# taleinat/fuzzysearch

Hardware: AMD Instinct MI355X
Metric: GB/s of sequence scanned at |p|=20 max_l_dist=2 (levenshtein_ngram path; two searches in flight: see value_sync for one synchronous call at a time) (higher is better)
Workload: dtype u8

## Files before the change

fuzzysearch_amd/_native.py:

```python
import ctypes
import os
import threading

_HERE = os.path.dirname(os.path.abspath(__file__))
LIB_PATH = os.environ.get("FUZZYSEARCH_HIP_LIB") or os.path.join(_HERE, "libfzhip.so")

FZ_OK, FZ_EINVAL, FZ_ENOMEM, FZ_EDEVICE, FZ_EUNSUPPORTED, FZ_EHALO, FZ_ETIMEOUT = 0, -1, -2, -3, -4, -5, -6
UINT64_MAX = (1 << 64) - 1

EXPORTED_SYMBOLS = (
    "fz_abi_version", "fz_last_error", "fz_device_count", "fz_create", "fz_destroy",
    "fz_seq_upload", "fz_seq_upload_shard", "fz_seq_new", "fz_seq_add_shard", "fz_seq_len", "fz_seq_release",
    "fz_search_exact", "fz_lev_ngrams", "fz_lev_ngrams_begin", "fz_lev_ngrams_end", "fz_subs_ngrams", "fz_generic_ngrams",
    "fz_subs_ngrams_begin", "fz_generic_ngrams_begin", "fz_search_end",
    "fz_lev_lp", "fz_subs_lp", "fz_generic_lp", "fz_subs_ngrams_any", "fz_subs_lp_any", "fz_generic_ngrams_any", "fz_generic_ngrams_consolidated",
    "fz_lev_ngrams_consolidated", "fz_subs_ngrams_best",
    "fz_stream_open", "fz_stream_buffer", "fz_stream_submit", "fz_stream_read_fd", "fz_stream_finish", "fz_stream_close",
    "fz_consolidate", "fz_group_best", "fz_merge_ranks", "fz_wire_pack", "fz_wire_merge", "fz_debug_launch_plan", "fz_debug_order_records", "fz_debug_order_records_bounded", "fz_debug_order_segments", "fz_stats", "fz_mem_info", "fz_set_timing", "fz_set_streams", "fz_device_ms", "fz_free",
    "fz_comm_unique_id", "fz_comm_init_rank", "fz_comm_init_all", "fz_comm_info", "fz_comm_set_collective",
    "fz_comm_allgather", "fz_comm_max_f64", "fz_comm_barrier", "fz_comm_destroy", "fz_comm_gather_ms", "fz_comm_backend", "fz_debug_reload_switches", "fz_debug_gather_merge", "fz_debug_scan_regions",
)


class FzMatch(ctypes.Structure):
    _fields_ = [("start", ctypes.c_int64), ("end", ctypes.c_int64),
                ("dist", ctypes.c_int32), ("block", ctypes.c_int32)]


class FzStats(ctypes.Structure):
    _fields_ = [("bytes_scanned", ctypes.c_uint64), ("ngram_hits", ctypes.c_uint64),
                ("raw_matches", ctypes.c_uint64), ("filter_ms", ctypes.c_double),
                ("verify_ms", ctypes.c_double), ("device_ms", ctypes.c_double),
                ("filter_launches", ctypes.c_uint32), ("n_devices", ctypes.c_uint32),
                ("verify_form", ctypes.c_uint32), ("reserved_", ctypes.c_uint32)]


FORM_NONE, FORM_FUSED_BAND, FORM_FUSED_CELLS, FORM_FUSED_BITS1, FORM_FUSED_BITS2, FORM_KERNEL, FORM_FUSED_BITS32 = range(7)


class HipEngineError(RuntimeError):
    """libfzhip.so missing / no usable gfx950 device / HIP runtime failure."""


class CollectiveTimeout(HipEngineError):
    """A collective of the context's communicator did not complete within FZ_COMM_TIMEOUT_MS (a rank never arrived)."""


_lib = None
_lib_lock = threading.Lock()


def load_library():
    global _lib
# ... 25 lines not shown
        L.fz_seq_upload_shard.argtypes = [vp, u8p, u64, u64, u64, u64, u64, ctypes.POINTER(vp)]
        L.fz_seq_new.restype = ci
        L.fz_seq_new.argtypes = [vp, u64, ctypes.POINTER(vp)]
        L.fz_seq_add_shard.restype = ci
        L.fz_seq_add_shard.argtypes = [vp, ci, u8p, u64, u64, u64, u64]
        L.fz_device_ms.restype = ci
        L.fz_device_ms.argtypes = [vp, ctypes.POINTER(ctypes.c_double), ci]
        L.fz_comm_unique_id.restype = ci
        L.fz_comm_unique_id.argtypes = [vp, u64]
        L.fz_comm_init_rank.restype = ci
        L.fz_comm_init_rank.argtypes = [vp, vp, ci, ci]
        L.fz_comm_init_all.restype = ci
        L.fz_comm_init_all.argtypes = [vp]
        L.fz_comm_info.restype = ci
        L.fz_comm_info.argtypes = [vp, ctypes.POINTER(ci), ctypes.POINTER(ci), ctypes.POINTER(ci)]
        L.fz_comm_set_collective.restype = ci
        L.fz_comm_set_collective.argtypes = [vp, ci]
        L.fz_comm_allgather.restype = ci
        L.fz_comm_allgather.argtypes = [vp, vp, u64, vp]
        L.fz_comm_max_f64.restype = ci
        L.fz_comm_max_f64.argtypes = [vp, ctypes.POINTER(ctypes.c_double)]
        L.fz_comm_barrier.restype = ci
        L.fz_comm_barrier.argtypes = [vp]
        L.fz_comm_destroy.restype = None
        L.fz_comm_destroy.argtypes = [vp]
        L.fz_debug_reload_switches.restype = None
        L.fz_debug_reload_switches.argtypes = []
        L.fz_comm_backend.restype = ci
        L.fz_comm_backend.argtypes = []
        L.fz_comm_gather_ms.restype = ci
        L.fz_comm_gather_ms.argtypes = [vp, ctypes.POINTER(ctypes.c_double)]
        L.fz_debug_scan_regions.restype = ci
        L.fz_debug_scan_regions.argtypes = [u64, u64, u32, ci, ctypes.c_double, ci, ctypes.POINTER(u32), ctypes.c_void_p]
        L.fz_debug_gather_merge.restype = ci
        L.fz_debug_gather_merge.argtypes = [ctypes.c_void_p, u32, u64, ctypes.c_void_p, u32, mpp, u64p, u64p]
        L.fz_seq_len.restype = u64
        L.fz_seq_len.argtypes = [vp]
        L.fz_seq_release.restype = None
        L.fz_seq_release.argtypes = [vp]
        L.fz_search_exact.restype = ci
        L.fz_search_exact.argtypes = [vp, vp, u8p, u32, u64, u64, ctypes.POINTER(u64p), u64p]
        L.fz_lev_ngrams.restype = ci
        L.fz_lev_ngrams.argtypes = [vp, vp, u8p, u32, u32, mpp, u64p]
        L.fz_lev_ngrams_begin.restype = ci
        L.fz_lev_ngrams_begin.argtypes = [vp, vp, u8p, u32, u32]
        L.fz_lev_ngrams_end.restype = ci
        L.fz_lev_ngrams_end.argtypes = [vp, mpp, u64p]
        L.fz_search_end.restype = ci
        L.fz_search_end.argtypes = [vp, mpp, u64p]
        L.fz_subs_ngrams_begin.restype = ci
        L.fz_subs_ngrams_begin.argtypes = [vp, vp, u8p, u32, u32]
        L.fz_generic_ngrams_begin.restype = ci
        L.fz_generic_ngrams_begin.argtypes = [vp, vp, u8p, u32, u32, u32, u32, u32, ci]
        L.fz_subs_ngrams.restype = ci
        L.fz_subs_ngrams.argtypes = [vp, vp, u8p, u32, u32, mpp, u64p]
        L.fz_generic_ngrams.restype = ci
        L.fz_generic_ngrams.argtypes = [vp, vp, u8p, u32, u32, u32, u32, u32, mpp, u64p]
        L.fz_lev_lp.restype = ci
        L.fz_lev_lp.argtypes = [vp, vp, u8p, u32, u32, mpp, u64p]
        L.fz_subs_lp.restype = ci
        L.fz_subs_lp.argtypes = [vp, vp, u8p, u32, u32, mpp, u64p]
        L.fz_generic_lp.restype = ci
        L.fz_generic_lp.argtypes = [vp, vp, u8p, u32, u32, u32, u32, u32, mpp, u64p]
        L.fz_lev_ngrams_consolidated.restype = ci
        L.fz_lev_ngrams_consolidated.argtypes = [vp, vp, u8p, u32, u32, mpp, u64p]
        L.fz_subs_ngrams_best.restype = ci
# ... 587 lines not shown
```

fuzzysearch_amd/csrc/fzhip.hip:

```cpp
#include <hip/hip_runtime.h>
#include <hip/hip_ext.h>
#include <rccl/rccl.h>
#include <dlfcn.h>

#include <algorithm>
#include <atomic>
#include <chrono>
#include <condition_variable>
#include <cstdarg>
#include <cstdio>
#include <cstdlib>
#include <cstring>
#include <functional>
#include <new>
#include <string>
#include <thread>
#include <unistd.h>
#include <map>
#include <mutex>
#include <vector>
#include <cassert>

#include "../../include/fzhip.h"
#include "fz_kernels.h"
// ... 110 lines not shown
    bool dedup_zeroed = false;
    uint64_t gen_dedup_arg = 0;
    bool dedup_used = false;
    bool gen_multi_used = false;
    uint64_t gen_rows_cap = 0;
    uint8_t *h_big = nullptr;
    uint64_t big_cap = 0;
    uint8_t *spare_alloc = nullptr;
    uint64_t spare_bytes = 0;
    uint64_t first_copy = 512;
    bool header_zeroed = false;
    bool verify_launched = false;
    int scan_end_event = 1;
    int verify_end_event = 2;
    uint8_t *stream_h[2] = {nullptr, nullptr};
    uint8_t *stream_d = nullptr;
    uint64_t stream_cap = 0, stream_d_bytes = 0;
    int n_cus = 256;
    uint64_t hit_cap_used = 0, rec_cap_used = 0;
    bool fused_used = false;
    uint32_t form_used = 0;
    bool timed = true;
    double last_filter_ms = 0;
    uint64_t fold_guess = 8192, fold_copied = 0;
    bool fold_direct = true;
    bool fold_was_direct = false;
    int lp_end_event = 2;
    uint8_t *d_pat = nullptr;
    uint64_t pat_cap = 0;
    int slot_id = 0;
    uint32_t launches_used = 0;
    hipStream_t stream_alt = nullptr;
    uint8_t *d_hdr_alt = nullptr;
    ncclComm_t comm = nullptr;
    int comm_rank = -1;
    hipStream_t comm_stream = nullptr;
    uint8_t *d_send[2] = {nullptr, nullptr};
    uint64_t send_cap = 0;
    uint8_t *d_recv = nullptr, *h_recv = nullptr;
    uint64_t recv_bytes = 0;
    hipEvent_t ev_snap[2] = {nullptr, nullptr}, ev_done = nullptr;
    bool snap_taken[2] = {false, false};
    struct Slot {
        hipEvent_t ev[4] = {nullptr, nullptr, nullptr, nullptr};
        uint8_t *h_stage = nullptr, *h_stage_dev = nullptr;
        bool last_direct = false, verify_launched = false, fused_used = false, timed = true;
        int scan_end_event = 1, verify_end_event = 2;
        uint64_t hit_cap_used = 0, rec_cap_used = 0;
        int slot_id = 1;
    } other;
    void swap_slot() {
        std::swap(slot_id, other.slot_id);
        for (int i = 0; i < 4; ++i) std::swap(ev[i], other.ev[i]);
        std::swap(h_stage, other.h_stage);
        std::swap(h_stage_dev, other.h_stage_dev);
        std::swap(last_direct, other.last_direct);
        std::swap(verify_launched, other.verify_launched);
        std::swap(timed, other.timed);
        std::swap(fused_used, other.fused_used);
        std::swap(scan_end_event, other.scan_end_event);
        std::swap(verify_end_event, other.verify_end_event);
        std::swap(hit_cap_used, other.hit_cap_used);
        std::swap(rec_cap_used, other.rec_cap_used);
    }
};

struct Shard {
    int dev = 0;
    uint8_t *d_alloc = nullptr;
    uint8_t *d_buf = nullptr;
    uint64_t alloc_bytes = 0;
    FzGeom geom{};
};

}

namespace {

struct DevWorkers {
    struct W {
        std::thread th;
        std::mutex mu;
        std::condition_variable cv;
        std::function<int()> job;
        std::atomic<uint64_t> posted{0}, done{0};
        int rc = 0;
        std::string err;
        bool stop = false;
    };
    std::vector<W *> ws;
    static constexpr long kSpinUs = 1500;

// ... 447 lines not shown
        nw[j] = j + 1 < steps ? per : T - per * (steps - 1);
        weight += f[j] * (double)nw[j];
    }
    const double share = (double)ntiles / weight;
    uint64_t at = 0, wg = 0;
    auto add = [&](uint64_t nwg, uint64_t tiles) {
        fa.reg_wg0[fa.nreg] = (uint32_t)wg; fa.reg_nwg[fa.nreg] = (uint32_t)nwg;
        fa.reg_tile0[fa.nreg] = at; fa.reg_end[fa.nreg] = at + tiles;
        ++fa.nreg; wg += nwg; at += tiles;
    };
    add(Gw - T, std::min<uint64_t>(ntiles, (uint64_t)(share * (double)(Gw - T) + 0.5)));
    for (int j = 0; j < steps; ++j) {
        const uint64_t left = ntiles - at;
        add(nw[j], j + 1 < steps ? std::min<uint64_t>(left, (uint64_t)(share * f[j] * (double)nw[j] + 0.5)) : left);
    }
    for (uint32_t r = 0; r < fa.nreg; ++r)
        if ((fa.reg_end[r] - fa.reg_tile0[r] + fa.reg_nwg[r] - 1) / fa.reg_nwg[r] >= FZ_TITER_MAX) { fa.nreg = 0; break; }
}

void plan_scan_regions(FzScanArgs &fa, uint64_t ntiles, uint64_t grid, uint32_t n_cus) {
    const int steps = sw().taper_steps;
    const double fmin = sw().taper_min;
    const int t_per_cu = sw().taper_wg_per_cu;
    plan_scan_regions(fa, ntiles, grid, n_cus, steps, fmin, t_per_cu);
}

struct ScanPlan {
    uint64_t ntiles = 0;
    uint32_t grid = 1;
    int wfg = 0;
    uint32_t form = FZ_FORM_NONE;
    uint32_t lds = 0;
    VerifyPlan vp;
};

ScanPlan plan_scan(const Search &q, const FzGeom &geom, uint32_t n_cus, bool with_verify, FzScanArgs &fa) {
    ScanPlan sp;
    const uint32_t L = q.plan.L;
    const uint32_t G = (uint32_t)q.plan.s.size();
    const bool in_memory = geom.seg_stride == 0;
    const uint64_t ntiles_all = (geom.buf_len + FZ_TILE_BYTES - 1) / FZ_TILE_BYTES;
    const uint64_t tile_lo = std::min<uint64_t>(ntiles_all, q.part_lo / FZ_TILE_BYTES);
    const uint64_t tile_hi = q.part_hi == ~0ull ? ntiles_all : std::min<uint64_t>(ntiles_all, (q.part_hi + FZ_TILE_BYTES - 1) / FZ_TILE_BYTES);
    const bool partial = tile_lo != 0 || tile_hi != ntiles_all;
    const uint64_t ntiles = sp.ntiles = tile_hi > tile_lo ? tile_hi - tile_lo : 0;
    constexpr uint64_t kTilesPerWg = 12;
    const uint64_t resident = (uint64_t)n_cus * 6;
    uint64_t max_grid = std::max<uint64_t>(resident, ntiles / kTilesPerWg);
    if (ntiles < resident * 120) {
        const uint64_t rounds = std::max<uint64_t>(1, (2 * ntiles + resident * 19 / 2) / (resident * 19));
        max_grid = resident * rounds;
    }
    const uint64_t min_grid = (ntiles + FZ_TITER_MAX - 1) / FZ_TITER_MAX;
    sp.grid = (uint32_t)std::max<uint64_t>(std::max<uint64_t>(1, min_grid), std::min<uint64_t>(ntiles, max_grid));
    plan_scan_regions(fa, ntiles, sp.grid, n_cus);
    if (partial) {
        fa.nreg = 1;
        fa.reg_wg0[0] = 0; fa.reg_nwg[0] = sp.grid; fa.reg_tile0[0] = tile_lo; fa.reg_end[0] = tile_hi;
    }

    const bool force_big = sw().force_big_verify;
    sp.vp = plan_verify(q);
    const VerifyPlan &vp = sp.vp;
    fa.band_w = q.mode == FZ_MODE_LEV ? 2 * q.k + 2 : 0;
    fa.win_dwords = (q.m + 2 * q.k + 6) / 4 + 1;
    const uint32_t mpad = (q.m + 15u) & ~15u;
    constexpr uint32_t target = 18u * 1024u;
    fa.vlanes = 64;
    uint32_t fused_lds;
    if (in_memory) {
        fa.win_pieces = (q.m + 2 * q.k + 3 + 15) / 16;
        fa.qcap = 128;
        while (fa.qcap > 64 && mpad + FZ_TABLE_BYTES + FZ_WAVES_PER_BLOCK * fz_wave_lds_pref_bytes(fa.qcap, fa.win_pieces) > target + 4096)
            fa.qcap >>= 1;
        fused_lds = mpad + FZ_TABLE_BYTES + FZ_WAVES_PER_BLOCK * fz_wave_lds_pref_bytes(fa.qcap, fa.win_pieces);
        if (fa.win_pieces * 16u + 16u > FZ_PAD_BACK) fused_lds = ~0u;
    } else {
        while (fa.vlanes > 16 && mpad + FZ_TABLE_BYTES + FZ_WAVES_PER_BLOCK * fz_wave_lds_bytes(fa.win_dwords, fa.band_w, fa.vlanes, true) > target)
            fa.vlanes >>= 1;
        fused_lds = mpad + FZ_TABLE_BYTES + FZ_WAVES_PER_BLOCK * fz_wave_lds_bytes(fa.win_dwords, fa.band_w, fa.vlanes, true);
    }
    fa.fused = (with_verify && !force_big && q.m <= FZ_MAX_M && q.k <= FZ_MAX_K && fused_lds <= kFusedLdsBudget &&
                (q.mode != FZ_MODE_LEV || q.k <= 4)) ? 1u : 0u;
    int bits_nw = 0;
    double per_tile = 0;
    {
        bool seen[256] = {false};
        uint32_t sigma = 0;
        for (uint32_t i = 0; i < q.m; ++i)
            if (!seen[q.p[i]]) { seen[q.p[i]] = true; ++sigma; }
        per_tile = 4096.0 * std::min<uint32_t>(G, FZ_MAX_BLOCKS_PER_LAUNCH);
        for (uint32_t i = 0; i < L && per_tile > 0.01; ++i) per_tile /= (double)std::max(2u, sigma);
    }
// ... 4 lines not shown
        bits_nw = q.m <= FZ_BITS_MAX_M(4) ? 4 : q.m <= FZ_BITS_MAX_M(1) ? 1 : 2;
        constexpr uint32_t budget = 26u * 1024u;
        const uint32_t fixed = mpad + FZ_TABLE_BYTES + FZ_PEQ_BYTES(bits_nw);
        uint32_t qc = sw().bits_qcap > 0 ? (uint32_t)sw().bits_qcap
                                         : (uint32_t)std::min(512.0, 64.0 + 32.0 * std::ceil(2.0 * per_tile / 32.0));
        while (qc > 64u && fixed + FZ_WAVES_PER_BLOCK * fz_wave_lds_pref_bytes(qc, fa.win_pieces) > budget) qc -= 32u;
        fa.qcap = qc;
        fused_lds = fixed + FZ_WAVES_PER_BLOCK * fz_wave_lds_pref_bytes(fa.qcap, fa.win_pieces);
        if (fused_lds > kFusedLdsBudget) bits_nw = 0;
        else fa.fused = 1u;
    }
    bool adapt_plain = false;
    if (!bits_nw && fa.fused && in_memory && with_verify && !sw().no_bits && per_tile > 16.0 && q.mode == FZ_MODE_SUBS) {
        const uint32_t fixed = mpad + FZ_TABLE_BYTES;
        uint32_t qc = sw().bits_qcap > 0 ? (uint32_t)sw().bits_qcap : (uint32_t)std::min(512.0, 64.0 + 32.0 * std::ceil(2.0 * per_tile / 32.0));
        while (qc > 64u && fixed + FZ_WAVES_PER_BLOCK * fz_wave_lds_pref_bytes(qc, fa.win_pieces) > target + 4096) qc -= 32u;
        if (fixed + FZ_WAVES_PER_BLOCK * fz_wave_lds_pref_bytes(qc, fa.win_pieces) <= kFusedLdsBudget) {
            adapt_plain = true;
            fa.qcap = qc;
            fused_lds = fixed + FZ_WAVES_PER_BLOCK * fz_wave_lds_pref_bytes(qc, fa.win_pieces);
        }
    }
    const bool no_wf_fuse = sw().no_wf_fuse;
    const uint32_t wf_fused_lds = mpad + FZ_TABLE_BYTES + FZ_WAVES_PER_BLOCK * fz_wave_lds_bytes(fz_wf_fused_dwords(fa.win_dwords, (uint32_t)vp.gw), 0, 1, true);
    const int wf32_env = sw().wf32;
    const bool wf_candidate = !bits_nw && !fa.fused && in_memory && with_verify && !force_big && !no_wf_fuse && vp.want_wf && !vp.big && vp.gw <= 32 &&
                              q.m <= FZ_MAX_M && wf_fused_lds <= target + 4096;
    const bool wf_fused = wf_candidate && (vp.gw == 16 || (wf32_env >= 0 ? wf32_env != 0 : per_tile > 0.1));
    if (wf_fused) { fa.fused = 1u; fused_lds = wf_fused_lds; fa.vlanes = 64; }
    sp.wfg = bits_nw ? bits_nw : adapt_plain ? 3 : wf_fused ? vp.gw : 0;
    sp.form = !with_verify ? FZ_FORM_NONE : bits_nw == 4 ? FZ_FORM_FUSED_BITS32 : bits_nw == 1 ? FZ_FORM_FUSED_BITS1 : bits_nw == 2 ? FZ_FORM_FUSED_BITS2
              : wf_fused ? FZ_FORM_FUSED_CELLS : fa.fused ? FZ_FORM_FUSED_BAND : FZ_FORM_KERNEL;
    sp.lds = fa.fused ? fused_lds : FZ_TABLE_BYTES + FZ_WAVES_PER_BLOCK * fz_wave_lds_bytes(0, 0, 64, true);
    return sp;
}

int enqueue_shard(fz_ctx *ctx, const Shard &sh, const Search &q, bool with_verify, bool copy_back = true) {
    DevState &d = lane_dev(ctx, sh.dev);
    HIP_TRY(hipSetDevice(d.device));
    unsigned long long *counters = reinterpret_cast<unsigned long long *>(d.d_out);
    FzRec *recs = reinterpret_cast<FzRec *>(d.d_out + kHeaderBytes);
    const bool no_direct = env_no_direct();
    const bool snapshot = copy_back && with_verify && q.collective;
    const bool direct = copy_back && d.direct && !no_direct && !snapshot && sh.geom.buf_len > 0 && !q.plan.s.empty();
    if (direct && with_verify) recs = reinterpret_cast<FzRec *>(d.h_stage_dev + kHeaderBytes);
    d.last_direct = direct;
    d.timed = ctx->timing;

    FzScanArgs fa;
    fill_common_args(fa, sh, q);
    const ScanPlan sp = plan_scan(q, sh.geom, (uint32_t)d.n_cus, with_verify, fa);
    const VerifyPlan &vp = sp.vp;
    const uint32_t L = q.plan.L;
    const uint32_t G = (uint32_t)q.plan.s.size();
    const uint64_t ntiles = sp.ntiles;
    const dim3 grid(sp.grid);
    if (q.mode == FZ_MODE_GENERIC && !with_verify) fa.gen_dedup = d.gen_dedup_arg;
    {
        int rc = stage_pattern(d, fa, q.p, q.m, with_verify && vp.big);
        if (rc) return rc;
    }
    const HashGeom hgeom(L);
    const int nwin = hgeom.nwin, dh = hgeom.dh;
    fa.d2 = nwin == 2 ? std::min<uint32_t>(L, 8) - 4 : 0;
    fa.mask1 = hgeom.mask1;
    fa.mask2 = 0xffffffffu;
    fa.hit_cap = d.hit_cap;
    fa.rec_cap = direct ? kHostRecs : d.rec_cap;
    const bool alt = ctx->streams == 2 && d.slot_id == 1 && fa.fused && direct && copy_back && !fa.pat_g && sh.geom.seg_stride == 0;
    const hipStream_t st = alt ? d.stream_alt : d.stream;
    if (alt) counters = reinterpret_cast<unsigned long long *>(d.d_hdr_alt);
    else {
        if (!d.header_zeroed) HIP_TRY(hipMemsetAsync(d.d_out, 0, kHeaderBytes, d.stream));
        d.header_zeroed = false;
    }

    const bool ext_events = copy_back && direct && !(with_verify && !fa.fused) && ntiles > 0 && G > 0;
    const bool attach = ntiles > 0 && G > 0;
    if (ctx->timing && !attach) HIP_TRY(hipEventRecord(d.ev[0], st));
    uint32_t launches = 0;
    for (uint32_t g0 = 0; g0 < G && ntiles > 0;) {
        uint32_t hash_k = 0, lut_shift = 0;
        const uint32_t nblk = choose_launch_blocks(q.p, q.plan.s.data(), g0, G, L, hash_k, lut_shift);
        fa.hash_k = hash_k;
        fa.lut_shift = lut_shift;
        fa.nblk = nblk;
        fa.g0 = g0;
        for (uint32_t b = 0; b < nblk; ++b) {
            const uint8_t *ng = q.p + q.plan.s[g0 + b];
            fa.A[b] = load_le32(ng, L) & fa.mask1;
            fa.B[b] = nwin == 2 ? load_le32(ng + fa.d2, 4) : 0;
            fa.H[b] = nwin == 2 ? fz_hash_windows(fa.A[b], load_le32(ng + dh, 3), fa.hash_k) : fz_hash_short(fa.A[b], fa.hash_k);
            fa.s[b] = q.plan.s[g0 + b];
            fz_block_range(q.mode, q.m, q.k, L, fa.s[b], fa.lo_rel[b], fa.hi_sub[b]);
        }
        const bool verify_follows = with_verify && !fa.fused;
        fa.host_hdr = (direct && !verify_follows && g0 + nblk >= G) ? reinterpret_cast<uint64_t>(d.h_stage_dev) : 0;
        fa.flags = q.any ? FZ_FLAG_ANY : 0u;
        for (uint32_t b = 1; b < nblk; ++b)
            for (uint32_t c = 0; c < b; ++c)
                if (fa.H[b] == fa.H[c]) fa.flags |= FZ_FLAG_DUP_HASHES;
        ScanKernel kern = scan_kernel(nwin, dh, fa.fused != 0, sh.geom.seg_stride != 0, fa.lut_shift == 2, sp.wfg);
// ... 310 lines not shown
        }
        NCCL_TRY(rccl_api()->GroupStart());
        for (DevState &d : ctx->devs)
            NCCL_TRY(rccl_api()->AllGather(d.d_send[d.slot_id], d.d_recv, bytes, ncclChar, d.comm, d.comm_stream));
        NCCL_TRY(rccl_api()->GroupEnd());
        DevState &d0 = ctx->devs[0];
        HIP_TRY(hipSetDevice(d0.device));
        HIP_TRY(hipMemcpyAsync(d0.h_recv, d0.d_recv, (uint64_t)world * bytes, hipMemcpyDeviceToHost, d0.comm_stream));
        HIP_TRY(hipEventRecord(d0.ev_done, d0.comm_stream));
        {
            int rcw = comm_wait(d0.comm_stream, "the all-gather of the ranks' records");
            if (rcw) { if (rcw == FZ_ETIMEOUT) ctx->comm_broken = true; return rcw; }
        }
        for (size_t i = 1; i < ctx->devs.size(); ++i) {
            HIP_TRY(hipSetDevice(ctx->devs[i].device));
            int rcw = comm_wait(ctx->devs[i].comm_stream, "the all-gather of the ranks' records");
            if (rcw) { if (rcw == FZ_ETIMEOUT) ctx->comm_broken = true; return rcw; }
        }
        uint64_t top = 0, total = 0;
        parse_gathered(d0.h_recv, world, bytes, ctx->gcap, seq->rank_lo.data(), recs, ctx->seg_ends, ctx->seg_order, &top, &total);
        if (top > ctx->gcap) {
            ctx->gcap = (top + top / 4 + 1023) / 1024 * 1024;
            continue;
        }
        ctx->stats.raw_matches = total;
        const uint64_t want = std::max<uint64_t>(1024, (top + top / 4 + 1023) / 1024 * 1024);
        if (want * 2 <= ctx->gcap) ctx->gcap = want;
        ctx->last_gather_ms = std::chrono::duration<double, std::milli>(std::chrono::steady_clock::now() - t_start).count();
        return FZ_OK;
    }
    return fail(FZ_EDEVICE, "all-gather capacity kept overflowing");
}

int search_enqueue(fz_ctx *ctx, fz_seq *seq, const Search &q, bool with_verify) {
    ctx->view = nullptr;
    ctx->view_n = 0;
    ctx->rows_ready = false;
    ctx->stats.filter_launches = 0;
    ctx->stats.bytes_scanned = ctx->stats.ngram_hits = ctx->stats.raw_matches = 0;
    ctx->stats.filter_ms = ctx->stats.verify_ms = ctx->stats.device_ms = 0;
    ctx->tref.clear();
    int rc = for_each_shard(ctx, seq, [ctx, seq, &q, with_verify](size_t si) { return enqueue_shard(ctx, seq->shards[si], q, with_verify); });
    if (rc) return rc;
    for (const Shard &sh : seq->shards) {
        const DevState &d = lane_dev(ctx, sh.dev);
        ctx->stats.filter_launches += d.launches_used;
        ctx->stats.verify_form = d.form_used;
    }
    return FZ_OK;
}

int emit_matches(const FzRec *recs, size_t cnt, uint32_t L, fz_match **out, uint64_t *n, uint64_t idx_bound, uint32_t blk_bound,
                 bool may_have_empty, std::vector<fz_match> *into);

int search_collect(fz_ctx *ctx, fz_seq *seq, const Search &q, bool with_verify, std::vector<FzRec> &recs,
                   std::vector<uint64_t> &hits) {
    const size_t ns = seq->shards.size();
    if (ctx->souts.size() < ns) ctx->souts.resize(ns);
    const bool order_rows = with_verify && !q.collective && ns > 1 && !q.any && seq->shards[0].geom.seg_stride == 0;
    for (int attempt = 0; attempt < 4; ++attempt) {
        recs.clear();
        hits.clear();
        ctx->rows_ready = false;
        ctx->stats.bytes_scanned = ctx->stats.ngram_hits = ctx->stats.raw_matches = 0;
        ctx->stats.filter_ms = ctx->stats.verify_ms = ctx->stats.device_ms = 0;
        ctx->tref.clear();
        Trace tr;
        ctx->seg_ends.clear();
        ctx->seg_order.clear();
        const uint32_t L = q.plan.L, nblk = (uint32_t)q.plan.s.size();
        const uint64_t nglob = seq->n;
        const bool collective = q.collective;
        int rc = for_each_shard(ctx, seq, [ctx, seq, with_verify, ns, collective, order_rows, L, nblk, nglob](size_t si) {
            ShardOut &so = ctx->souts[si];
            int r = collect_shard(ctx, seq->shards[si], with_verify, ns == 1, so, collective);
// ... 637 lines not shown
    }
    return FZ_OK;
}

int fz_create(const int *device_ids, int n_devices, fz_ctx **out) {
    if (!out) return fail(FZ_EINVAL, "null argument");
    *out = nullptr;
    int count = 0;
    hipError_t e = hipGetDeviceCount(&count);
    if (e != hipSuccess || count <= 0)
        return fail(FZ_EDEVICE, "no HIP device available (%s)", e == hipSuccess ? "count = 0" : hipGetErrorString(e));
    (void)hipSetDeviceFlags(hipDeviceScheduleSpin);
    (void)hipGetLastError();
    std::vector<int> ids;
    if (!device_ids || n_devices <= 0) ids.push_back(0);
    else ids.assign(device_ids, device_ids + n_devices);
    fz_ctx *ctx = new (std::nothrow) fz_ctx();
    if (!ctx) return fail(FZ_ENOMEM, "out of memory");
    for (int id : ids) {
        if (id < 0 || id >= count) { fz_destroy(ctx); return fail(FZ_EINVAL, "device id %d out of range (have %d)", id, count); }
        hipDeviceProp_t prop;
        if (hipGetDeviceProperties(&prop, id) != hipSuccess) { fz_destroy(ctx); return fail(FZ_EDEVICE, "hipGetDeviceProperties failed"); }
        if (strncmp(prop.gcnArchName, "gfx950", 6) != 0) {
            fz_destroy(ctx);
            return fail(FZ_EDEVICE, "device %d is %s; libfzhip is built for gfx950 (MI355X) only", id, prop.gcnArchName);
        }
        ctx->devs.emplace_back();
        DevState &d = ctx->devs.back();
        d.device = id;
        d.n_cus = prop.multiProcessorCount > 0 ? prop.multiProcessorCount : 256;
        int rc = devstate_init(d);
        if (rc) { fz_destroy(ctx); return rc; }
    }
    if (ctx->devs.size() > 1 && !sw().no_dev_threads) {
        ctx->workers = new (std::nothrow) DevWorkers(ctx->devs.size());
        if (!ctx->workers) { fz_destroy(ctx); return fail(FZ_ENOMEM, "out of memory"); }
    }
    *out = ctx;
    return FZ_OK;
}

void fz_destroy(fz_ctx *ctx) {
    if (!ctx) return;
    delete ctx->workers;
    ctx->workers = nullptr;
    while (!ctx->live.empty()) {
        for (DevState &d : ctx->devs) { (void)hipSetDevice(d.device); if (d.stream) (void)hipStreamSynchronize(d.stream); }
        fz_seq_release(ctx->live.back());
    }
    comm_teardown(ctx);
    for (DevState &d : ctx->devs) devstate_destroy(d);
    for (DevState &d : ctx->devs2) devstate_destroy(d);
    delete ctx;
}

static int upload_one(fz_ctx *ctx, int dev_index, const uint8_t *host_buf, const FzGeom &geom, Shard &sh) {
    DevState &d = ctx->devs[dev_index];
    HIP_TRY(hipSetDevice(d.device));
    const uint64_t tiles = (geom.buf_len + FZ_TILE_BYTES - 1) / FZ_TILE_BYTES;
    const uint64_t body = std::max<uint64_t>(1, tiles) * FZ_TILE_BYTES;
    sh.dev = dev_index;
    sh.alloc_bytes = FZ_PAD_FRONT + body + FZ_PAD_BACK;
    sh.geom = geom;
    if (d.spare_alloc && d.spare_bytes >= sh.alloc_bytes && d.spare_bytes <= 4 * sh.alloc_bytes + (1u << 20)) {
        sh.d_alloc = d.spare_alloc;
        sh.alloc_bytes = d.spare_bytes;
// ... 306 lines not shown
    if (ctx && ctx->npend >= 2) return fail(FZ_EINVAL, "two searches are already in flight on this context");
    const bool generic = kind == FZ_MODE_GENERIC;
    if (ctx && ctx->npend == 1 && (ctx->pend[0].kind == FZ_MODE_GENERIC) != generic)
        return fail(FZ_EINVAL, "generic searches and Levenshtein / substitutions-only searches cannot be in flight together");
    if (!ctx || !p || m == 0) return fail(FZ_EINVAL, "bad ctx / empty subsequence");
    fz_ctx::Pending &pd = ctx->pend[ctx->npend];
    pd.pattern.assign(p, p + m);
    pd.seq = seq;
    pd.m = m;
    pd.k = k;
    pd.kind = kind;
    pd.max_subs = max_subs; pd.max_ins = max_ins; pd.max_dels = max_dels;
    pd.consolidated = consolidated;
    pd.lane = 0;
    Search q;
    int rc = pending_plan(ctx, pd, q);
    if (rc) return rc;
    memset(&ctx->stats, 0, sizeof ctx->stats); ctx->tref.clear();
    ctx->stats.n_devices = (uint32_t)ctx->devs.size();
    const bool second = ctx->npend == 1;
    pd.launched = true;
    if (generic) {
        pd.lane = second ? 1 - ctx->pend[0].lane : 0;
        if (pd.lane == 1) { rc = ensure_lane2(ctx); if (rc) return rc; }
        std::vector<FzGenRec> none;
        ctx->lane = pd.lane;
        rc = run_generic(ctx, seq, q, none, 1);
        ctx->lane = 0;
        if (rc) return rc;
    } else {
        if (second && !ctx->snapshot) for (const DevState &d : ctx->devs) if (!d.direct || env_no_direct()) pd.launched = false;
        if (pd.launched) {
            if (second) for (DevState &d : ctx->devs) d.swap_slot();
            rc = search_enqueue(ctx, seq, q, true);
            if (second) for (DevState &d : ctx->devs) d.swap_slot();
            if (rc) return rc;
        }
    }
    ++ctx->npend;
    return FZ_OK;
}

int fz_lev_ngrams_begin(fz_ctx *ctx, fz_seq *seq, const uint8_t *p, uint32_t m, uint32_t k) {
    return pending_begin(ctx, seq, p, m, FZ_MODE_LEV, k, 0, 0, 0, false);
}

int fz_subs_ngrams_begin(fz_ctx *ctx, fz_seq *seq, const uint8_t *p, uint32_t m, uint32_t k) {
    return pending_begin(ctx, seq, p, m, FZ_MODE_SUBS, k, 0, 0, 0, false);
}

int fz_generic_ngrams_begin(fz_ctx *ctx, fz_seq *seq, const uint8_t *p, uint32_t m, uint32_t max_subs, uint32_t max_ins,
                            uint32_t max_dels, uint32_t max_l, int consolidated) {
    return pending_begin(ctx, seq, p, m, FZ_MODE_GENERIC, max_l, max_subs, max_ins, max_dels, consolidated != 0);
}

int fz_search_end(fz_ctx *ctx, fz_match **out, uint64_t *n) {
    if (!ctx || !out || !n) return fail(FZ_EINVAL, "null argument");
    *out = nullptr; *n = 0;
    if (!ctx->npend) return fail(FZ_EINVAL, "no search in flight");
    fz_ctx::Pending &pd = ctx->pend[0];
    Search q;
    int rc = pending_plan(ctx, pd, q);
    if (pd.kind == FZ_MODE_GENERIC) {
        std::vector<FzGenRec> recs_vec;
        ctx->lane = pd.lane;
        if (rc == FZ_OK) rc = run_generic(ctx, pd.seq, q, recs_vec, 2);
        if (rc == FZ_OK) rc = generic_exchange(ctx, recs_vec);
// ... 457 lines not shown
        NCCL_TRY(rccl_api()->AllReduce(tmp, tmp, 1, ncclDouble, ncclMax, d.comm, d.comm_stream));
        HIP_TRY(hipMemcpyAsync(value, tmp, sizeof(double), hipMemcpyDeviceToHost, d.comm_stream));
        return comm_wait(d.comm_stream, "an all-reduce over the job's ranks");
    };
    rc = body();
    if (rc == FZ_ETIMEOUT) ctx->comm_broken = true;
    else (void)hipFree(tmp);
    return rc;
}

int fz_comm_barrier(fz_ctx *ctx) {
    if (ctx) for (DevState &d : ctx->devs) { (void)hipSetDevice(d.device); (void)hipStreamSynchronize(d.stream); (void)hipStreamSynchronize(d.stream_alt); }
    double one = 1.0;
    return fz_comm_max_f64(ctx, &one);
}

void fz_debug_reload_switches(void) { switches_storage() = read_switches(); }

int fz_comm_backend(void) { return !rccl_api()->ok ? 0 : rccl_api()->stand_in ? 2 : 1; }

int fz_comm_gather_ms(fz_ctx *ctx, double *ms) {
    if (!ctx || !ms) return fail(FZ_EINVAL, "null argument");
    *ms = ctx->last_gather_ms;
    return FZ_OK;
}

int fz_debug_scan_regions(uint64_t ntiles, uint64_t grid, uint32_t n_cus, int steps, double fmin, int wg_per_cu, uint32_t *n_regions,
                          uint64_t *table) {
    if (!n_regions || !table) return fail(FZ_EINVAL, "null argument");
    static FzScanArgs fa;
    static std::mutex mu;
    std::lock_guard<std::mutex> lk(mu);
    plan_scan_regions(fa, ntiles, grid, n_cus, steps, fmin, wg_per_cu);
    *n_regions = fa.nreg;
    for (uint32_t r = 0; r < fa.nreg; ++r) {
        table[4 * r] = fa.reg_wg0[r]; table[4 * r + 1] = fa.reg_nwg[r]; table[4 * r + 2] = fa.reg_tile0[r]; table[4 * r + 3] = fa.reg_end[r];
    }
    return FZ_OK;
}

int fz_debug_gather_merge(const void *blocks, uint32_t world, uint64_t cap, const uint64_t *own_lo, uint32_t L, fz_match **out,
                          uint64_t *n_out, uint64_t *need_cap) {
    if (!blocks || !out || !n_out || !need_cap || world == 0) return fail(FZ_EINVAL, "null argument");
    *out = nullptr; *n_out = 0; *need_cap = 0;
    std::vector<FzRec> recs;
    std::vector<size_t> seg_ends;
    std::vector<uint32_t> seg_order;
    uint64_t top = 0, total = 0;
    parse_gathered(static_cast<const uint8_t *>(blocks), (int)world, kHeaderBytes + cap * sizeof(FzRec), cap, own_lo, recs, seg_ends,
                   seg_order, &top, &total);
    if (top > cap) { *need_cap = (top + top / 4 + 1023) / 1024 * 1024; return FZ_OK; }
    return emit_matches_segments(nullptr, recs.data(), seg_ends, seg_order, L, out, n_out, 0, 0, true);
}

}

namespace {

struct LpRec { int64_t start, end; int32_t dist; uint64_t step; uint64_t w0; uint32_t seq; };

constexpr uint32_t kLpStarts = 256;

int run_lp(fz_ctx *ctx, fz_seq *seq, const Search &q, uint32_t lp_kind, std::vector<LpRec> &out) {
    if ((uint64_t)q.m + 2ull * q.k + kLpStarts > 65535ull)
        return fail(FZ_EUNSUPPORTED, "linear-programming route: len(subsequence) + 2 * max_l_dist + %u = %llu exceeds 65535 (16-bit window coordinates)",
                    kLpStarts, (unsigned long long)q.m + 2ull * q.k + kLpStarts);
// ... 1203 lines not shown
```

include/fzhip.h:

```cpp
#ifndef FZHIP_H
#define FZHIP_H

#include <stdint.h>

#ifdef __cplusplus
extern "C" {
#endif

#define FZ_ABI_VERSION 1

#define FZ_OK          0
#define FZ_EINVAL     -1
#define FZ_ENOMEM     -2
#define FZ_EDEVICE    -3
#define FZ_EUNSUPPORTED -4
#define FZ_EHALO      -5
#define FZ_ETIMEOUT   -6

typedef struct fz_ctx fz_ctx;
typedef struct fz_seq fz_seq;

typedef struct {
    int64_t start, end;
    int32_t dist;
// ... 94 lines not shown

int fz_group_best(const fz_match *in, uint64_t n, fz_match **out, uint64_t *n_out);

int fz_merge_ranks(const fz_match *const *parts, const uint64_t *counts, const uint64_t *block_counts,
                   uint32_t world, uint32_t nb, fz_match *out);

#define FZ_WIRE_HEADER_ROWS 65
int fz_wire_pack(const fz_match *in, uint64_t n, uint64_t cap_rows, void *dst);
int fz_wire_merge(const void *recv, uint32_t world, uint64_t rows_per_rank, uint64_t cap_rows,
                  fz_match *out, uint64_t out_cap, uint64_t *n_out, uint64_t *max_count);

typedef struct fz_stream fz_stream;
int  fz_stream_open(fz_ctx *ctx, uint32_t mode, const uint8_t *p, uint32_t m, uint32_t max_subs, uint32_t max_ins,
                    uint32_t max_dels, uint32_t k, uint64_t seg_stride, uint32_t seg_pre, uint32_t seg_post,
                    uint64_t batch_bytes, fz_stream **out);
int  fz_stream_buffer(fz_stream *st, uint8_t **host, uint64_t *capacity);
int  fz_stream_submit(fz_stream *st, uint64_t nbytes, int last);
int  fz_stream_read_fd(fz_stream *st, int fd, int64_t offset, int threads, uint64_t *total);
int  fz_stream_finish(fz_stream *st, fz_match **out, uint32_t **seg, uint64_t *n);
void fz_stream_close(fz_stream *st);

void fz_debug_reload_switches(void);

int fz_debug_launch_plan(const uint8_t *p, uint32_t m, uint32_t L, uint32_t *out, uint32_t cap, uint32_t *n_launches);

int fz_debug_order_records(const void *recs, uint64_t n, uint32_t L, fz_match **out, uint64_t *n_out);
int fz_debug_order_records_bounded(const void *recs, uint64_t n, uint32_t L, uint64_t idx_bound, uint32_t blk_bound,
                                   fz_match **out, uint64_t *n_out);
int fz_debug_order_segments(const void *recs, const uint64_t *seg_ends, uint32_t n_segments, uint32_t L, fz_match **out, uint64_t *n_out);

int fz_debug_scan_regions(uint64_t ntiles, uint64_t grid, uint32_t n_cus, int steps, double fmin, int wg_per_cu, uint32_t *n_regions,
                          uint64_t *table);

int fz_debug_gather_merge(const void *blocks, uint32_t world, uint64_t cap, const uint64_t *own_lo, uint32_t L, fz_match **out,
                          uint64_t *n_out, uint64_t *need_cap);

int  fz_stats(fz_ctx *ctx, fz_stats_t *out);
int  fz_mem_info(fz_ctx *ctx, uint64_t *free_bytes, uint64_t *total_bytes);
int  fz_set_timing(fz_ctx *ctx, int on);
int  fz_set_streams(fz_ctx *ctx, int n);
int  fz_device_ms(fz_ctx *ctx, double *filter_ms, int cap);
void fz_free(void *p);

#ifdef __cplusplus
}
#endif
#endif
```

Baseline: 4860.

## Plan overlapped second search with untapered grid and alternate stream by default

When a second search is enqueued behind a first on a single device, the scan plan now marks it as overlapped. For that case it uses a larger tiles-per-workgroup grid cap and skips the tapered region schedule, because the concurrent search already fills the chip. It also sets two streams by default on single-device contexts and chooses the alternate stream according to whether the other slot is already on it. A debug export for inspecting the scan plan is added as well. The risk is that the untapered grid leaves a load-imbalanced tail when the two searches do not actually overlap.

```diff
diff --git a/fuzzysearch_amd/_native.py b/fuzzysearch_amd/_native.py
--- a/fuzzysearch_amd/_native.py
+++ b/fuzzysearch_amd/_native.py
@@ -19,6 +19,7 @@
     "fz_consolidate", "fz_group_best", "fz_merge_ranks", "fz_wire_pack", "fz_wire_merge", "fz_debug_launch_plan", "fz_debug_order_records", "fz_debug_order_records_bounded", "fz_debug_order_segments", "fz_stats", "fz_mem_info", "fz_set_timing", "fz_set_streams", "fz_device_ms", "fz_free",
     "fz_comm_unique_id", "fz_comm_init_rank", "fz_comm_init_all", "fz_comm_info", "fz_comm_set_collective",
     "fz_comm_allgather", "fz_comm_max_f64", "fz_comm_barrier", "fz_comm_destroy", "fz_comm_gather_ms", "fz_comm_backend", "fz_debug_reload_switches", "fz_debug_gather_merge", "fz_debug_scan_regions",
+    "fz_debug_scan_plan",
 )
 
 
@@ -110,6 +111,10 @@
         L.fz_comm_gather_ms.argtypes = [vp, ctypes.POINTER(ctypes.c_double)]
         L.fz_debug_scan_regions.restype = ci
         L.fz_debug_scan_regions.argtypes = [u64, u64, u32, ci, ctypes.c_double, ci, ctypes.POINTER(u32), ctypes.c_void_p]
+        if hasattr(L, "fz_debug_scan_plan"):
+            L.fz_debug_scan_plan.restype = ci
+            L.fz_debug_scan_plan.argtypes = [ctypes.c_char_p, u32, u32, u64, u32, ci, ctypes.POINTER(u32), ctypes.POINTER(u32),
+                                             ctypes.POINTER(ci), ctypes.POINTER(u32), ctypes.c_void_p]
         L.fz_debug_gather_merge.restype = ci
         L.fz_debug_gather_merge.argtypes = [ctypes.c_void_p, u32, u64, ctypes.c_void_p, u32, mpp, u64p, u64p]
         L.fz_seq_len.restype = u64
diff --git a/fuzzysearch_amd/csrc/fzhip.hip b/fuzzysearch_amd/csrc/fzhip.hip
--- a/fuzzysearch_amd/csrc/fzhip.hip
+++ b/fuzzysearch_amd/csrc/fzhip.hip
@@ -166,6 +166,7 @@
     uint32_t launches_used = 0;
     hipStream_t stream_alt = nullptr;
     uint8_t *d_hdr_alt = nullptr;
+    bool on_alt = false;
     ncclComm_t comm = nullptr;
     int comm_rank = -1;
     hipStream_t comm_stream = nullptr;
@@ -178,7 +179,7 @@
     struct Slot {
         hipEvent_t ev[4] = {nullptr, nullptr, nullptr, nullptr};
         uint8_t *h_stage = nullptr, *h_stage_dev = nullptr;
-        bool last_direct = false, verify_launched = false, fused_used = false, timed = true;
+        bool last_direct = false, verify_launched = false, fused_used = false, timed = true, on_alt = false;
         int scan_end_event = 1, verify_end_event = 2;
         uint64_t hit_cap_used = 0, rec_cap_used = 0;
         int slot_id = 1;
@@ -192,6 +193,7 @@
         std::swap(verify_launched, other.verify_launched);
         std::swap(timed, other.timed);
         std::swap(fused_used, other.fused_used);
+        std::swap(on_alt, other.on_alt);
         std::swap(scan_end_event, other.scan_end_event);
         std::swap(verify_end_event, other.verify_end_event);
         std::swap(hit_cap_used, other.hit_cap_used);
@@ -705,9 +707,10 @@
     uint32_t form = FZ_FORM_NONE;
     uint32_t lds = 0;
     VerifyPlan vp;
+    bool overlapped = false;
 };
 
-ScanPlan plan_scan(const Search &q, const FzGeom &geom, uint32_t n_cus, bool with_verify, FzScanArgs &fa) {
+ScanPlan plan_scan(const Search &q, const FzGeom &geom, uint32_t n_cus, bool with_verify, bool shares_chip, FzScanArgs &fa) {
     ScanPlan sp;
     const uint32_t L = q.plan.L;
     const uint32_t G = (uint32_t)q.plan.s.size();
@@ -717,21 +720,6 @@
     const uint64_t tile_hi = q.part_hi == ~0ull ? ntiles_all : std::min<uint64_t>(ntiles_all, (q.part_hi + FZ_TILE_BYTES - 1) / FZ_TILE_BYTES);
     const bool partial = tile_lo != 0 || tile_hi != ntiles_all;
     const uint64_t ntiles = sp.ntiles = tile_hi > tile_lo ? tile_hi - tile_lo : 0;
-    constexpr uint64_t kTilesPerWg = 12;
-    const uint64_t resident = (uint64_t)n_cus * 6;
-    uint64_t max_grid = std::max<uint64_t>(resident, ntiles / kTilesPerWg);
-    if (ntiles < resident * 120) {
-        const uint64_t rounds = std::max<uint64_t>(1, (2 * ntiles + resident * 19 / 2) / (resident * 19));
-        max_grid = resident * rounds;
-    }
-    const uint64_t min_grid = (ntiles + FZ_TITER_MAX - 1) / FZ_TITER_MAX;
-    sp.grid = (uint32_t)std::max<uint64_t>(std::max<uint64_t>(1, min_grid), std::min<uint64_t>(ntiles, max_grid));
-    plan_scan_regions(fa, ntiles, sp.grid, n_cus);
-    if (partial) {
-        fa.nreg = 1;
-        fa.reg_wg0[0] = 0; fa.reg_nwg[0] = sp.grid; fa.reg_tile0[0] = tile_lo; fa.reg_end[0] = tile_hi;
-    }
-
     const bool force_big = sw().force_big_verify;
     sp.vp = plan_verify(q);
     const VerifyPlan &vp = sp.vp;
@@ -802,10 +790,30 @@
     sp.form = !with_verify ? FZ_FORM_NONE : bits_nw == 4 ? FZ_FORM_FUSED_BITS32 : bits_nw == 1 ? FZ_FORM_FUSED_BITS1 : bits_nw == 2 ? FZ_FORM_FUSED_BITS2
               : wf_fused ? FZ_FORM_FUSED_CELLS : fa.fused ? FZ_FORM_FUSED_BAND : FZ_FORM_KERNEL;
     sp.lds = fa.fused ? fused_lds : FZ_TABLE_BYTES + FZ_WAVES_PER_BLOCK * fz_wave_lds_bytes(0, 0, 64, true);
+    sp.overlapped = shares_chip && fa.fused && in_memory && !partial && q.m <= FZ_MAX_M && !vp.big;
+
+    constexpr uint64_t kTilesPerWg = 12;
+    const uint64_t resident = (uint64_t)n_cus * 6;
+    uint64_t max_grid = std::max<uint64_t>(resident, ntiles / kTilesPerWg);
+    if (ntiles < resident * 120) {
+        const uint64_t rounds = std::max<uint64_t>(1, (2 * ntiles + resident * 19 / 2) / (resident * 19));
+        max_grid = resident * rounds;
+    }
+    constexpr uint64_t kTilesPerWgOverlapped = 16;
+    constexpr bool kTaperOverlapped = false;
+    if (sp.overlapped) max_grid = std::max<uint64_t>(resident, ntiles / kTilesPerWgOverlapped);
+    const uint64_t min_grid = (ntiles + FZ_TITER_MAX - 1) / FZ_TITER_MAX;
+    sp.grid = (uint32_t)std::max<uint64_t>(std::max<uint64_t>(1, min_grid), std::min<uint64_t>(ntiles, max_grid));
+    if (!sp.overlapped || kTaperOverlapped) plan_scan_regions(fa, ntiles, sp.grid, n_cus);
+    else fa.nreg = 0;
+    if (partial) {
+        fa.nreg = 1;
+        fa.reg_wg0[0] = 0; fa.reg_nwg[0] = sp.grid; fa.reg_tile0[0] = tile_lo; fa.reg_end[0] = tile_hi;
+    }
     return sp;
 }
 
-int enqueue_shard(fz_ctx *ctx, const Shard &sh, const Search &q, bool with_verify, bool copy_back = true) {
+int enqueue_shard(fz_ctx *ctx, const Shard &sh, const Search &q, bool with_verify, bool copy_back = true, bool behind = false) {
     DevState &d = lane_dev(ctx, sh.dev);
     HIP_TRY(hipSetDevice(d.device));
     unsigned long long *counters = reinterpret_cast<unsigned long long *>(d.d_out);
@@ -819,7 +827,7 @@
 
     FzScanArgs fa;
     fill_common_args(fa, sh, q);
-    const ScanPlan sp = plan_scan(q, sh.geom, (uint32_t)d.n_cus, with_verify, fa);
+    const ScanPlan sp = plan_scan(q, sh.geom, (uint32_t)d.n_cus, with_verify, behind && ctx->streams == 2 && direct, fa);
     const VerifyPlan &vp = sp.vp;
     const uint32_t L = q.plan.L;
     const uint32_t G = (uint32_t)q.plan.s.size();
@@ -837,7 +845,9 @@
     fa.mask2 = 0xffffffffu;
     fa.hit_cap = d.hit_cap;
     fa.rec_cap = direct ? kHostRecs : d.rec_cap;
-    const bool alt = ctx->streams == 2 && d.slot_id == 1 && fa.fused && direct && copy_back && !fa.pat_g && sh.geom.seg_stride == 0;
+    if (sp.overlapped && fa.pat_g) return fail(FZ_EDEVICE, "internal: an overlapped scan with the pattern staged in HBM");
+    const bool alt = sp.overlapped && !d.other.on_alt;
+    d.on_alt = alt;
     const hipStream_t st = alt ? d.stream_alt : d.stream;
     if (alt) counters = reinterpret_cast<unsigned long long *>(d.d_hdr_alt);
     else {
@@ -1214,7 +1224,7 @@
     return fail(FZ_EDEVICE, "all-gather capacity kept overflowing");
 }
 
-int search_enqueue(fz_ctx *ctx, fz_seq *seq, const Search &q, bool with_verify) {
+int search_enqueue(fz_ctx *ctx, fz_seq *seq, const Search &q, bool with_verify, bool behind = false) {
     ctx->view = nullptr;
     ctx->view_n = 0;
     ctx->rows_ready = false;
@@ -1222,7 +1232,9 @@
     ctx->stats.bytes_scanned = ctx->stats.ngram_hits = ctx->stats.raw_matches = 0;
     ctx->stats.filter_ms = ctx->stats.verify_ms = ctx->stats.device_ms = 0;
     ctx->tref.clear();
-    int rc = for_each_shard(ctx, seq, [ctx, seq, &q, with_verify](size_t si) { return enqueue_shard(ctx, seq->shards[si], q, with_verify); });
+    int rc = for_each_shard(ctx, seq, [ctx, seq, &q, with_verify, behind](size_t si) {
+        return enqueue_shard(ctx, seq->shards[si], q, with_verify, true, behind);
+    });
     if (rc) return rc;
     for (const Shard &sh : seq->shards) {
         const DevState &d = lane_dev(ctx, sh.dev);
@@ -1926,6 +1938,7 @@
         int rc = devstate_init(d);
         if (rc) { fz_destroy(ctx); return rc; }
     }
+    ctx->streams = ctx->devs.size() == 1 ? 2 : 1;
     if (ctx->devs.size() > 1 && !sw().no_dev_threads) {
         ctx->workers = new (std::nothrow) DevWorkers(ctx->devs.size());
         if (!ctx->workers) { fz_destroy(ctx); return fail(FZ_ENOMEM, "out of memory"); }
@@ -2298,7 +2311,7 @@
         if (second && !ctx->snapshot) for (const DevState &d : ctx->devs) if (!d.direct || env_no_direct()) pd.launched = false;
         if (pd.launched) {
             if (second) for (DevState &d : ctx->devs) d.swap_slot();
-            rc = search_enqueue(ctx, seq, q, true);
+            rc = search_enqueue(ctx, seq, q, true, second);
             if (second) for (DevState &d : ctx->devs) d.swap_slot();
             if (rc) return rc;
         }
@@ -2822,6 +2835,31 @@
     static std::mutex mu;
     std::lock_guard<std::mutex> lk(mu);
     plan_scan_regions(fa, ntiles, grid, n_cus, steps, fmin, wg_per_cu);
+    *n_regions = fa.nreg;
+    for (uint32_t r = 0; r < fa.nreg; ++r) {
+        table[4 * r] = fa.reg_wg0[r]; table[4 * r + 1] = fa.reg_nwg[r]; table[4 * r + 2] = fa.reg_tile0[r]; table[4 * r + 3] = fa.reg_end[r];
+    }
+    return FZ_OK;
+}
+
+int fz_debug_scan_plan(const uint8_t *p, uint32_t m, uint32_t k, uint64_t buf_len, uint32_t n_cus, int shares_chip, uint32_t *grid,
+                       uint32_t *form, int *overlapped, uint32_t *n_regions, uint64_t *table) {
+    if (!p || !grid || !form || !overlapped || !n_regions || !table || m == 0 || m / (k + 1) == 0 || n_cus == 0)
+        return fail(FZ_EINVAL, "bad argument");
+    Search q;
+    q.mode = FZ_MODE_LEV; q.m = m; q.k = k; q.p = p;
+    q.plan.L = m / (k + 1);
+    for (uint32_t s = 0; s + q.plan.L <= m; s += q.plan.L) q.plan.s.push_back(s);
+    FzGeom geom{};
+    geom.buf_len = buf_len;
+    static FzScanArgs fa;
+    static std::mutex mu;
+    std::lock_guard<std::mutex> lk(mu);
+    memset(&fa, 0, sizeof fa);
+    const ScanPlan sp = plan_scan(q, geom, n_cus, true, shares_chip != 0, fa);
+    *grid = sp.grid;
+    *form = sp.form;
+    *overlapped = sp.overlapped ? 1 : 0;
     *n_regions = fa.nreg;
     for (uint32_t r = 0; r < fa.nreg; ++r) {
         table[4 * r] = fa.reg_wg0[r]; table[4 * r + 1] = fa.reg_nwg[r]; table[4 * r + 2] = fa.reg_tile0[r]; table[4 * r + 3] = fa.reg_end[r];
diff --git a/include/fzhip.h b/include/fzhip.h
--- a/include/fzhip.h
+++ b/include/fzhip.h
@@ -150,6 +150,9 @@
 int fz_debug_scan_regions(uint64_t ntiles, uint64_t grid, uint32_t n_cus, int steps, double fmin, int wg_per_cu, uint32_t *n_regions,
                           uint64_t *table);
 
+int fz_debug_scan_plan(const uint8_t *p, uint32_t m, uint32_t k, uint64_t buf_len, uint32_t n_cus, int shares_chip, uint32_t *grid,
+                       uint32_t *form, int *overlapped, uint32_t *n_regions, uint64_t *table);
+
 int fz_debug_gather_merge(const void *blocks, uint32_t world, uint64_t cap, const uint64_t *own_lo, uint32_t L, fz_match **out,
                           uint64_t *n_out, uint64_t *need_cap);
 
```

After: 5291, median of 6. +8.9%, better.
